# yeyupiaoling/PPASR

Hardware: AMD Instinct MI355X
Metric: audio-seconds/s (RTF^-1) Conformer-streaming fbank, batch32 per GPU, ctc_greedy (higher is better)
Workload: dtype f32; 1 GPU; configs[1]: Conformer streaming (configs/conformer.yml), fbank-80, 32 x 10 s utterances per GPU, V=4233, ctc_greedy, features resident in HBM -> token ids + scores on device; global_batch=32, frames=1000, decoder=ctc_greedy, parallelism=utterance-dp1, pipelined=False, gemm=f32

## Files before the change

### ppasr_amd/csrc/encode_common.h

```cpp
#pragma once

struct RaggedPlan {
  bool skip;
  const int64_t* lens;
  int rc;
  bool rate_changes;
  int mul0;
  int slack(int mul) const { return rate_changes && mul == mul0 ? 2 * (rc + 4) + rc + 8 : rc + 4; }
  PadSkip at(int Tcur, int mul) const {
    PadSkip ps;
    if (skip) {
      ps.lens = lens;
      ps.Tp = Tcur;
      ps.mul = mul;
      ps.slack = slack(mul);
    }
    return ps;
  }
  int attn_pad_skip(const PadSkip& ps) const { return skip ? ps.slack + 1 : 0; }
};

struct BlockTables {
  struct Tab { int Ti, R; int* tab; } tabs[4];
  int n = 0, B;
  bool fits, on;
  size_t off, cap;
  int* base;
  hipStream_t st;
  BlockTables(bool skip, int B_, int M, float* stats, hipStream_t st_)
      : B(B_), off(((size_t)B_ + 2 + 15) / 16 * 16), cap(2 * (((size_t)M + 63) / 64 * 64)), base(reinterpret_cast<int*>(stats)), st(st_) {
    fits = (size_t)B + 2 <= cap / 2;
    on = skip && fits && block_tables_enabled();
  }
  int* tile_tab() const { return fits ? base : nullptr; }
  PadSkip make(PadSkip p, int Tcur, int R) {
    const size_t len = 1 + ((size_t)B * Tcur + R - 1) / R;
    if (!on || n == 4 || off + len > cap) return p;
    int* t = base + off;
    launch_block_table(p, B * Tcur, R, t, st);
    tabs[n++] = Tab{Tcur, R, t};
    off += (len + 15) / 16 * 16;
    p.tab = t;
    return p;
  }
  PadSkip with_table(PadSkip p, int Tcur, int R) {
    for (int k = 0; k < n; ++k)
      if (tabs[k].Ti == Tcur && tabs[k].R == R) {
        p.tab = tabs[k].tab;
        return p;
      }
    return make(p, Tcur, R);
  }
};

struct Taps {
  float* buf;
  size_t cap;
  hipStream_t st;
  size_t off = 0;
  void operator()(const float* src, size_t n_floats) {
    if (buf && off + n_floats <= cap)
      (void)hipMemcpyAsync(buf + off, src, n_floats * sizeof(float), hipMemcpyDeviceToDevice, st);
    off += n_floats;
  }
};

struct NoSpans {
  template <typename Fn>
  void operator()(int, Fn&& fn) const { fn(); }
};

template <typename Spans>
inline void front4_fused(const ppasr_model_s* h, const float* feats, int B, int T, const PadSkip& ps, int* tile_tab,
                         bool scale_before_bias, int embed_slices, const PadSkip& ps_embed, float* y1, float* y2, float* xa,
                         hipStream_t st, Spans&& spans) {
  const auto fd = h->front_dims(T);
  const int F = h->desc.input_dim, T1 = fd.T1, F1 = h->F1, Tp = fd.Tp, F2 = h->F2;
  const bool il4 = h->desc.input_layer == 0;
  const f32x4* conv2_h3 = h->gemm_mode == PPASR_GEMM_F16X3 ? h->conv2_w_h3 : nullptr;
  const bool conv12 = il4 && !conv2_h3 && conv12_enabled(h) && conv12_supported(h->front, F, F2);
  if (!conv12) spans(0, [&] { launch_conv1(feats, h->front, y1, B, T, F, T1, F1, st, ps); });
  spans(1, [&] {
    if (conv12) launch_conv12(feats, h->front, y2, B, T, F, Tp, F2, st, ps, tile_tab);
    else if (il4 && !conv2_h3 && conv2_quad_supported(h->front)) launch_conv2_quad(y1, h->front, y2, B, T1, F1, Tp, F2, st, ps, tile_tab);
    else launch_conv2(y1, h->front, y2, B, T1, F1, Tp, F2, st, ps, tile_tab, il4 ? conv2_h3 : nullptr);
  });
  spans(2, [&] {
    launch_embed(y2, h->front, xa, B * Tp, F2 * kD, sqrtf((float)kD), scale_before_bias, st, ps_embed, embed_slices, y1,
                 conv2_h3 ? h->embed_w_h3 : nullptr);
  });
}

inline ppasr_status memory_out(const ppasr_model_s* h, const float* x, const float* g, const float* b, int M, int D,
                               const PadSkip& ps, hipStream_t st) {
  if (!h->memory_out) return PPASR_OK;
  if ((size_t)M * D > h->memory_floats) return fail(PPASR_ENOSPACE, "memory buffer too small (ppasr_set_memory_out)");
  launch_memory_out(x, g, b, h->memory_out, M, D, ps, st);
  return PPASR_OK;
}

template <typename Spans>
inline ppasr_status fused_head_tail(const ppasr_model_s* h, const float* x, float* probs, float* logits, int32_t* frame_argmax,
                                    float* frame_maxprob, float* ws, const WsLayout& wl, int B, int M, int slices,
                                    const PadSkip& ps, hipStream_t st, Spans&& spans) {
  if (ppasr_status ms = memory_out(h, x, h->head.ln_g, h->head.ln_b, M, kD, ps, st)) return ms;
  float* lg = logits ? logits : probs;
  int32_t* fa = frame_argmax ? frame_argmax : reinterpret_cast<int32_t*>(ws + wl.fa);
  float* fp = frame_maxprob ? frame_maxprob : ws + wl.fp;
  spans(7, [&] {
    const bool head_h3 = h->gemm_mode == PPASR_GEMM_F16X3 && h->head_w_h3;
    HeadW hw = h->head;
    if (head_h3) hw.w = h->head_w_h3;
    launch_ctc_head(x, hw, lg, fa, fp, ws + wl.rmax, ws + wl.rsum, M, st, ps, slices, ws + wl.y1, head_h3);
  });
  if (probs) {
    if (logits) HIP_TRY(hipMemcpyAsync(probs, logits, (size_t)M * h->head.V * sizeof(float), hipMemcpyDeviceToDevice, st));
    launch_softmax_from_stats(probs, ws + wl.rmax, ws + wl.rsum, M, h->head.V, st, ps);
  }
  if (ps.lens) launch_zero_pad_rows(probs, logits, fa, fp, ps.lens, B, ps.Tp, ps.mul, h->head.V, st);
  HIP_TRY(hipGetLastError());
  return PPASR_OK;
}

struct LayerRoute {
  int form;
  int S;
  bool fuse_attn;
  bool h3, h3s;
};
inline bool fuse_rows(const ppasr_model_s* h, int rows) {
  constexpr int fuse_min_blocks = 128;
  return ffn_split_for(h, rows) == 1 && (h->ffn_split == 0 || (rows + kRows - 1) / kRows > fuse_min_blocks);
}
inline LayerRoute layer_route(const ppasr_model_s* h, int B, int Ti, int mul, int slack, bool skip, int layer) {
  const int Mi = B * Ti;
  LayerRoute r;
  const int rows = (!h->taps && conv_ffn_16_supported(h->layer_ks[layer], Ti)) ? row_block_for(h, B, Ti, mul, slack, skip) : 32;
  const bool r16 = rows == 16 && h->ffn_split < 0;
  r.fuse_attn = !r16 && h->layer_group[layer] == 1 && h->desc.attention_heads == 4 && !h->taps && fuse_rows(h, Mi);
  r.S = r16 ? 1 : ffn_split_for(h, Mi);
  const bool w16 = rows == kW16 && r.S == 1;
  r.form = r16 ? 16 : w16 ? kW16 : 32;
  r.h3 = h->h3_layers() && !r16 && !w16 && r.S == 1;
  r.h3s = h->h3_layers() && r.S > 1;
  return r;
}
```

### ppasr_amd/csrc/front_fused.hip

```cpp
#include <utility>

#include "conformer_kernels.h"
#include "launch.h"

namespace ppasr {

namespace {
constexpr int kGroupRow[5] = {2, 0, 1, 4, 3};
constexpr int kTapCol[5] = {2, 0, 1, 4, 3};
constexpr int kFactor[5] = {2, 0, 1, 3, 1};
constexpr int quad_slab(int t) { return 4 * kFactor[t / 5] + kFactor[t % 5]; }
constexpr int quad_target(int t) {
  const int g = t / 5, k = t % 5;
  if (g == 0) return k == 0 ? 4 : k <= 2 ? 5 : 4;
  const int a = (g == 1 || g == 2) ? 0 : 2;
  return k == 0 ? (a == 0 ? 5 : 4) : k <= 2 ? a : a + 1;
}
constexpr int quad_fold_src(int t) {
  return t == 1 || t == 5 || t == 21 || t == 23 ? 4 : t == 3 || t == 11 || t == 13 ? 5 : -1;
}
constexpr int quad_fold_mask(int t) {
  return t == 1 ? 0xf : t == 3 ? 0x5 : t == 5 ? 0xa : t == 11 ? 0x2 : t == 13 ? 0x1 : t == 21 ? 0x8 : t == 23 ? 0x4 : 0;
}
constexpr bool quad_fold_clear(int t) { return t == 1 || t == 3 || t == 5 || t == 13 || t == 23; }
static_assert(quad_target(0) == 4 && quad_target(2) == 5 && quad_target(10) == 5 && quad_target(12) == 0 &&
                  quad_target(14) == 1 && quad_target(20) == 4 && quad_target(22) == 2 && quad_target(24) == 3,
              "chunk targets");

template <typename Fn, int... I>
__device__ __forceinline__ void static_for(std::integer_sequence<int, I...>, Fn&& fn) {
  (fn(std::integral_constant<int, I>{}), ...);
}

__host__ __device__ inline int quad_xs_stride(int F, int Q) { return F > 8 * Q + 3 ? F : 8 * Q + 3; }
}

template <bool FROM_Y1>
__device__ __forceinline__ void conv2_quad_body(const float* __restrict__ src, const FrontW& fw, float* __restrict__ out,
                                                int T, int F, int Tp, int F2, int M, int m0, const PadSkip& ps,
                                                const int* __restrict__ tile_tab) {
  constexpr int BP = 32, KC = 128, LD = KC + 4, G = KC / 8, NL = 2, N_CHUNKS = 25;
  constexpr int SLOT = BP * LD;
  const int P = (Tp + 1) >> 1;
  const int Q = (F2 + 1) >> 1;
  int r0 = m0 + blockIdx.x * BP, Mlim = M;
  if (tile_tab) {
    const int t = blockIdx.x, nb = tile_tab[0];
    const int* pre = tile_tab + 1;
    if (t >= pre[nb]) return;
    int lo = 0, hi = nb;
    while (hi - lo > 1) {
      const int mid = (lo + hi) >> 1;
      if (pre[mid] <= t) lo = mid;
      else hi = mid;
    }
    const int S = ps.Tp * ps.unit;
    r0 = lo * S + (t - pre[lo]) * BP;
    Mlim = min(M, (lo + 1) * S);
  } else if (pad_block_skippable(ps, r0, BP, M)) {
    return;
  }
  extern __shared__ __attribute__((aligned(16))) float smem[];
  float* const slot0 = smem;
  float* const slot1 = smem + SLOT;
  f32x4* const y2s = reinterpret_cast<f32x4*>(smem + 2 * SLOT);
  float* const w1s = smem + 2 * SLOT + 5 * NL * 4 * kThreads;
  float* const xs = w1s + 10 * 256;
  const int tid = threadIdx.x, lane = lane_id(), wave = wave_id();
  constexpr int tile_stride = 2 * 16 * G * 64;
  const f32x4* wbase = fw.conv2_wp + (size_t)wave * tile_stride;
  auto seg = [&](int h, int slab) { return wbase + (size_t)(16 * h + slab) * G * 64; };
  BRing<1> ring;
  ring_prime(ring, seg(0, quad_slab(0)), 0);
  const int c4 = tid & 31, rbase = tid >> 5;
  const int bp0 = r0 / Q;
  const int FX = quad_xs_stride(F, Q);
  uint32_t pb = 0;
  int yrow[FROM_Y1 ? NL : 1], yp4[FROM_Y1 ? NL : 1], yq4[FROM_Y1 ? NL : 1];
  if constexpr (!FROM_Y1) {
    for (int idx = tid; idx < 10 * 256; idx += kThreads) w1s[idx] = idx < 9 * 256 ? fw.conv1_w[idx] : fw.conv1_b[idx - 9 * 256];
    const int nbp = (min(r0 + BP, Mlim) - 1) / Q - bp0 + 1;
    for (int idx = tid; idx < nbp * 11 * FX; idx += kThreads) {
      const int fr_row = idx / FX, f = idx - fr_row * FX;
      const int bpl = fr_row / 11, fr = fr_row - 11 * bpl;
      const int bp = bp0 + bpl, b = bp / P, p = bp - b * P;
      const int t = min(8 * p + fr, T - 1);
      xs[idx] = f < F ? (src[((size_t)b * T + t) * F + f] - fw.cmvn_mean[f]) * fw.cmvn_istd[f] : 0.f;
    }
#pragma unroll
    for (int i = 0; i < NL; ++i) {
      const int m = r0 + rbase + 16 * i;
      const int bp = m / Q, q = m - bp * Q;
      const uint32_t v = m < Mlim ? (uint32_t)((bp - bp0) * 11 * FX + 8 * q) : 0xffffu;
      pb |= v << (16 * i);
    }
  } else {
#pragma unroll
    for (int i = 0; i < NL; ++i) {
      const int m = r0 + rbase + 16 * i;
      const int bp = m / Q, q = m - bp * Q, b = bp / P, p = bp - b * P;
      yrow[i] = b * T + 4 * p;
      yp4[i] = 4 * p;
      yq4[i] = m < Mlim ? 4 * q : -1;
    }
  }
  auto pbase = [&](int i) { return (int)((pb >> (16 * i)) & 0xffffu); };
  const int lds_off0 = rbase * LD + 4 * c4;
  float xv[9];
  f32x4 wv[3], bv, ya, yv;
  auto y1_step = [&](int i, int h, int r, int c, int step) {
    const int cc = h * 128 + 4 * c4;
    if constexpr (!FROM_Y1) {
      if (step == 0) {
        const int o = pbase(i);
        const float* p = xs + (o == 0xffff ? 0 : o) + 2 * r * FX + 2 * c;
#pragma unroll
        for (int ii = 0; ii < 3; ++ii)
#pragma unroll
          for (int jj = 0; jj < 3; ++jj) xv[ii * 3 + jj] = p[ii * FX + jj];
        ya = f32x4{0.f, 0.f, 0.f, 0.f};
      } else {
#pragma unroll
        for (int j = 3 * (step - 1); j < 3 * step; ++j)
#pragma unroll
          for (int e = 0; e < 4; ++e) ya[e] = fmaf(wv[j % 3][e], xv[j], ya[e]);
        if (step == 3) {
          ya += bv;
#pragma unroll
          for (int e = 0; e < 4; ++e) ya[e] = pbase(i) != 0xffff ? fmaxf(ya[e], 0.f) : 0.f;
        }
      }
      if (step < 3) {
#pragma unroll
        for (int j = 0; j < 3; ++j) wv[j] = *reinterpret_cast<const f32x4*>(w1s + (3 * step + j) * 256 + cc);
        if (step == 2) bv = *reinterpret_cast<const f32x4*>(w1s + 9 * 256 + cc);
      }
    } else {
      if (step == 0) {
        yv = f32x4{0.f, 0.f, 0.f, 0.f};
        if (yq4[i] >= 0 && yp4[i] + r < T && yq4[i] + c < F)
          yv = *reinterpret_cast<const f32x4*>(src + ((size_t)(yrow[i] + r) * F + yq4[i] + c) * 256 + cc);
      } else if (step == 3) {
        ya = yv;
      }
    }
  };
  auto put = [&](float* buf, int i, const f32x4& v) { *reinterpret_cast<f32x4*>(buf + lds_off0 + i * 16 * LD) = v; };
  auto y2row = [&](int c, int i) -> f32x4& { return y2s[(c * NL + i) * kThreads + tid]; };
  f32x4 z2[NL];
  auto build = [&](auto nc, int g, int h, float* buf) {
    constexpr int n = decltype(nc)::value, grp = n / 5, k = n % 5, r = kGroupRow[grp], c = kTapCol[k];
    const int i = g >> 2, step = g & 3;
    y1_step(i, h, r, c, step);
    if (step != 3) return;
    f32x4 v = ya;
    if constexpr (grp == 0) y2row(c, i) = ya;
    if constexpr (grp == 1 || grp == 3) v = ya - y2row(c, i);
    if constexpr (k == 0) {
      z2[i] = v;
      put(buf, i, v);
    } else if constexpr (k == 1 || k == 3) {
      put(buf, i, v - z2[i]);
    } else {
      put(buf, i, v);
    }
  };
  f32x16 acc[6][1][1];
#pragma unroll
  for (int a = 0; a < 6; ++a) acc_zero(acc[a]);
  auto fold = [&](auto tc, int g) {
    constexpr int t = decltype(tc)::value, fs = quad_fold_src(t), mask = quad_fold_mask(t);
    if constexpr (fs >= 0) {
      const int j = g - 4 * NL;
      int seen = 0;
#pragma unroll
      for (int o = 0; o < 4; ++o) {
        if (!((mask >> o) & 1)) continue;
        if (seen++ == j) {
#pragma unroll
          for (int e = 0; e < 16; ++e) asm volatile("v_add_f32 %0, %0, %1" : "+v"(acc[o][0][0][e]) : "v"(acc[fs][0][0][e]));
        }
      }
      if (quad_fold_clear(t) && j == 4) acc_zero(acc[fs]);
    }
  };
  __syncthreads();
#pragma unroll
  for (int g = 0; g < 4 * NL; ++g) {
    build(std::integral_constant<int, 0>{}, g, 0, slot0);
    __builtin_amdgcn_sched_barrier(0);
  }
  __syncthreads();
  for (int h = 0; h < 2; ++h) {
    asm volatile("" : "+s"(wbase));
    if constexpr (!FROM_Y1) {
      asm volatile("" : "+v"(pb));
    } else {
#pragma unroll
      for (int i = 0; i < NL; ++i) asm volatile("" : "+v"(yrow[i]), "+v"(yp4[i]), "+v"(yq4[i]));
    }
    static_for(std::make_integer_sequence<int, N_CHUNKS>{}, [&](auto tc) {
      constexpr int t = decltype(tc)::value;
      float* const cur = ((t + h) & 1) ? slot1 : slot0;
      float* const nxb = ((t + h) & 1) ? slot0 : slot1;
      const f32x4* nseg = t + 1 < N_CHUNKS ? seg(h, quad_slab(t + 1)) : (h == 0 ? seg(1, quad_slab(0)) : nullptr);
      auto side = [&](int g) {
        if (g < 4 * NL) {
          if constexpr (t + 1 < N_CHUNKS) build(std::integral_constant<int, t + 1>{}, g, h, nxb);
          else if (h == 0) build(std::integral_constant<int, 0>{}, g, 1, nxb);
        } else {
          fold(tc, g);
        }
      };
      rb_gemm<1, 1, G, kPF, decltype(side)>(cur, LD, seg(h, quad_slab(t)), 0, nseg, 0, ring, acc[quad_target(t)], side);
      __syncthreads();
    });
  }
  const int col = wave * 32 + (lane & 31);
  const float b2 = fw.conv2_b[col];
#pragma unroll
  for (int r = 0; r < 16; ++r) {
    const int m = r0 + acc_row(r, lane);
    if (m >= Mlim) continue;
    const int bp = m / Q, q = m - bp * Q, b = bp / P, t0 = 2 * (bp - b * P), f0 = 2 * q;
    float* o = out + ((size_t)(b * Tp + t0) * F2 + f0) * 256 + col;
    const bool f1 = f0 + 1 < F2, t1 = t0 + 1 < Tp;
    o[0] = fmaxf(acc[0][0][0][r] + b2, 0.f);
    if (f1) o[256] = fmaxf(acc[1][0][0][r] + b2, 0.f);
    if (t1) o[(size_t)F2 * 256] = fmaxf(acc[2][0][0][r] + b2, 0.f);
    if (t1 && f1) o[(size_t)F2 * 256 + 256] = fmaxf(acc[3][0][0][r] + b2, 0.f);
  }
}

__global__ __launch_bounds__(kThreads) void k_conv12(const float* __restrict__ feats, FrontW fw, float* __restrict__ out,
                                                     int T, int F, int Tp, int F2, int M, int m0, PadSkip ps,
                                                     const int* __restrict__ tile_tab) {
  conv2_quad_body<false>(feats, fw, out, T, F, Tp, F2, M, m0, ps, tile_tab);
}
__global__ __launch_bounds__(kThreads) void k_conv2_pair(const float* __restrict__ y1, FrontW fw, float* __restrict__ out,
                                                         int T1, int F1, int Tp, int F2, int M, int m0, PadSkip ps,
                                                         const int* __restrict__ tile_tab) {
  conv2_quad_body<true>(y1, fw, out, T1, F1, Tp, F2, M, m0, ps, tile_tab);
}

static int quad_tile_pairs(int Q) { return 31 / Q + 2; }
static size_t quad_lds(bool fused, int F, int F2) {
  const int Q = (F2 + 1) / 2;
  return ((size_t)2 * 32 * 132 + (size_t)5 * 2 * 4 * 512 + (fused ? (size_t)10 * 256 + (size_t)quad_tile_pairs(Q) * 11 * quad_xs_stride(F, Q) : 0)) *
         sizeof(float);
}
bool conv2_quad_supported(const FrontW& fw) { return fw.conv2_wp && fw.conv2_k == 3 && fw.conv2_s == 2; }
bool conv12_supported(const FrontW& fw, int F, int F2) {
  const int Q = (F2 + 1) / 2;
  return conv2_quad_supported(fw) && F2 >= 1 && quad_lds(true, F, F2) <= 160 * 1024 &&
         (size_t)quad_tile_pairs(Q) * 11 * quad_xs_stride(F, Q) < 0xffff;
}

void launch_tile_prefix(const PadSkip& ps, int B, int BM, int* tab, hipStream_t st);

static void launch_quad(bool fused, const float* src, const FrontW& fw, float* y2, int B, int T, int F, int Tp, int F2,
                        hipStream_t st, const PadSkip& ps_frames, int* tile_scratch) {
  const int P = (Tp + 1) / 2, Q = (F2 + 1) / 2;
  PadSkip ps = ps_frames;
  ps.Tp = P;
  ps.mul = 2 * ps_frames.mul;
  ps.slack = (ps_frames.slack + 1) / 2;
  ps.unit = Q;
  const int M = B * P * Q;
  const int* no_tab = nullptr;
#define QUAD(GRID, TAB)                                                                                                  \
  do {                                                                                                                 \
    if (fused)                                                                                                         \
      PPASR_LAUNCH(k_conv12, dim3(GRID), dim3(kThreads), quad_lds(true, F, F2), st, src, fw, y2, T, F, Tp, F2, M, 0, ps, \
                   TAB);                                                                                               \
    else                                                                                                               \
      PPASR_LAUNCH(k_conv2_pair, dim3(GRID), dim3(kThreads), quad_lds(false, F, F2), st, src, fw, y2, T, F, Tp, F2, M, 0, \
                   ps, TAB);                                                                                           \
  } while (0)
  if (ps.lens && tile_scratch) {
    launch_tile_prefix(ps, B, 32, tile_scratch, st);
    QUAD(B * ((P * Q + 31) / 32), (const int*)tile_scratch);
    return;
  }
  QUAD((M + 31) / 32, no_tab);
#undef QUAD
}

void launch_conv12(const float* feats, const FrontW& fw, float* y2, int B, int T, int F, int Tp, int F2, hipStream_t st,
                   const PadSkip& ps_frames, int* tile_scratch) {
  launch_quad(true, feats, fw, y2, B, T, F, Tp, F2, st, ps_frames, tile_scratch);
}
void launch_conv2_quad(const float* y1, const FrontW& fw, float* y2, int B, int T1, int F1, int Tp, int F2, hipStream_t st,
                       const PadSkip& ps_frames, int* tile_scratch) {
  launch_quad(false, y1, fw, y2, B, T1, F1, Tp, F2, st, ps_frames, tile_scratch);
}

hipError_t configure_front_fused_kernels() {
  hipError_t e;
#define SET_LDS(fn)                                                                                              \
  e = hipFuncSetAttribute(reinterpret_cast<const void*>(fn), hipFuncAttributeMaxDynamicSharedMemorySize, 160 * 1024); \
  if (e != hipSuccess) return e;
  SET_LDS(k_conv12);
  SET_LDS(k_conv2_pair);
#undef SET_LDS
  return hipSuccess;
}

}
```

### ppasr_amd/csrc/front_kernels.hip

```cpp
#include <algorithm>
#include <cstdlib>

#include "conformer_kernels.h"
#include "launch.h"
#include "phases.h"
#include "h3.h"

#include <math.h>

namespace ppasr {
#ifdef PPASR_PHASE_TS
}
extern "C" __attribute__((visibility("default"))) int ppasr_debug_read_wave_ts_front(long long* out) {
  return (int)hipMemcpyFromSymbol(out, HIP_SYMBOL(ppasr::g_wave_ts), sizeof(long long) * 512);
}
namespace ppasr {
#endif

__global__ void k_posproj(const float* __restrict__ pe, const float* __restrict__ wpos,
                          const float* __restrict__ bpos, float* __restrict__ ptab, int max_len, int d) {
  int pos = blockIdx.x;
  int n = threadIdx.x;
  __shared__ float row[1024];
  row[n] = pe[(size_t)pos * d + n];
// ... 80 lines not shown
  constexpr int BM = 32 * MT;
  int r0_map = 0, Mlim = M;
  if (tile_tab) {
    const int t = blockIdx.x, nb = tile_tab[0];
    const int* pre = tile_tab + 1;
    if (t >= pre[nb]) return;
    int lo = 0, hi = nb;
    while (hi - lo > 1) {
      const int mid = (lo + hi) >> 1;
      if (pre[mid] <= t) lo = mid;
      else hi = mid;
    }
    const int S = ps.Tp * ps.unit;
    r0_map = lo * S + (t - pre[lo]) * BM;
    Mlim = min(M, (lo + 1) * S);
  } else if (ps.tab) {
    const int blk = pad_block_of(ps, BM, M);
    if (blk < 0) return;
    r0_map = blk * BM;
  } else if (pad_block_skippable(ps, m0 + blockIdx.x * BM, BM, M)) {
    return;
  }
  constexpr int LD = H3 ? (KC + 8) / 2 : KC + 4;
  constexpr int LDH = KC + 8, PLANE = BM * LDH;
  constexpr int BUF = H3 ? PLANE : BM * LD;
  constexpr int F4_PER_ROW = KC / 4;
  constexpr int NL = BM * F4_PER_ROW / kThreads;
  constexpr int G = KC / 8;
  extern __shared__ __attribute__((aligned(16))) float smem[];
  const int tid = threadIdx.x, lane = lane_id(), wave = wave_id();
  const int r0 = (tile_tab || ps.tab) ? r0_map : m0 + blockIdx.x * BM;
  const int tile_stride = n_chunks * G * 64;
  const int kc0 = (int)((long long)blockIdx.z * n_chunks / gridDim.z), kc1 = (int)((long long)(blockIdx.z + 1) * n_chunks / gridDim.z);
  const f32x4* wbase = wp + (size_t)(blockIdx.y * kWaves + wave) * tile_stride;
  BRing<1> ring;
  ring_prime(ring, wbase + (size_t)kc0 * G * 64, 0);
  const float* tile_base = src.base(min(r0, M - 1));
  const __amdgpu_buffer_rsrc_t rs_a = wstream_rsrc(tile_base);
  int voff[NL];
  int lds_off[NL];
#pragma unroll
  for (int i = 0; i < NL; ++i) {
    int idx = tid + kThreads * i;
    int row = idx / F4_PER_ROW, c4 = idx - row * F4_PER_ROW;
    int m = r0 + row;
    voff[i] = (m < Mlim) ? (int)((src.base(m) - tile_base) * sizeof(float)) + 16 * c4 : 0x7fffffff;
    lds_off[i] = H3 ? row * LDH + 4 * c4 : row * LD + 4 * c4;
  }
  f32x4 stg[NL];
  auto load_chunk = [&](int kc) {
    const int soff = (int)(src.chunk_off(kc) * sizeof(float));
#pragma unroll
    for (int i = 0; i < NL; ++i) stg[i] = wstream_load(rs_a, voff[i], soff);
  };
  bool bad = false;
  auto write_piece = [&](float* buf, int i) {
    _Float16* pl = reinterpret_cast<_Float16*>(buf);
    f16x4 hi, lo;
    h3_split4(stg[i] * kH3Sa, hi, lo, bad);
    *reinterpret_cast<f16x4*>(pl + lds_off[i]) = hi;
    *reinterpret_cast<f16x4*>(pl + PLANE + lds_off[i]) = lo;
  };
  auto write_chunk = [&](float* buf) {
    if constexpr (H3) {
#pragma unroll
      for (int i = 0; i < NL; ++i) write_piece(buf, i);
    } else {
#pragma unroll
      for (int i = 0; i < NL; ++i) *reinterpret_cast<f32x4*>(buf + lds_off[i]) = stg[i];
    }
  };
  f32x16 acc[MT][1];
  acc_zero(acc);
  load_chunk(kc0);
  write_chunk(smem + (kc0 & 1) * BUF);
  __syncthreads();
  for (int kc = kc0; kc < kc1; ++kc) {
    float* cur = smem + (kc & 1) * BUF;
    float* nxt = smem + ((kc + 1) & 1) * BUF;
    const bool more = kc + 1 < kc1;
    if (more) load_chunk(kc + 1);
    const f32x4* seg = wbase + (size_t)kc * G * 64;
    if (MT == 4 && kc < 8) PPASR_WAVE_TS(32 + 4 * kc);
    if constexpr (H3) {
      constexpr int KS = KC / 16, PER = (NL + KS - 1) / KS;
      auto side = [&](int ks) {
        if (more) {
#pragma unroll
          for (int j = 0; j < PER; ++j)
            if (ks * PER + j < NL) write_piece(nxt, ks * PER + j);
        }
      };
      rb_gemm_h3_rows<MT, KS>(reinterpret_cast<const _Float16*>(cur), LDH, PLANE, seg, more ? seg + G * 64 : nullptr, ring, acc,
                              side);
    } else {
      rb_gemm<MT, 1, G>(cur, LD, seg, 0, more ? seg + G * 64 : nullptr, 0, ring, acc);
    }
    if (MT == 4 && kc < 8) PPASR_WAVE_TS(33 + 4 * kc);
    if constexpr (!H3) {
      if (more) write_chunk(nxt);
    }
    if (MT == 4 && kc < 8) PPASR_WAVE_TS(34 + 4 * kc);
    __syncthreads();
    if (MT == 4 && kc < 8) PPASR_WAVE_TS(35 + 4 * kc);
  }
  if constexpr (H3) {
    h3_note(bad);
#pragma unroll
    for (int mt = 0; mt < MT; ++mt) acc[mt][0] *= kH3Inv;
  }
  const int col = blockIdx.y * 256 + wave * 32 + (lane & 31);
  if (gridDim.z > 1) {
    float* po = out + (size_t)blockIdx.z * M * ldc;
#pragma unroll
    for (int mt = 0; mt < MT; ++mt)
#pragma unroll
      for (int r = 0; r < 16; ++r) {
        int m = r0 + mt * 32 + acc_row(r, lane);
        if (m < Mlim && col < n_valid) po[(size_t)m * ldc + col] = acc[mt][0][r];
      }
    return;
  }
  const float bv = bias[col];
#pragma unroll
  for (int mt = 0; mt < MT; ++mt)
#pragma unroll
    for (int r = 0; r < 16; ++r) {
      int m = r0 + mt * 32 + acc_row(r, lane);
      float v = SB ? acc[mt][0][r] * scale + bv : (acc[mt][0][r] + bv) * scale;
      if (RELU) v = fmaxf(v, 0.f);
      if (m < Mlim && col < n_valid) out[(size_t)m * ldc + col] = v;
    }
}
template <int MT, int KC, bool RELU, bool SB, typename Src>
__global__ __launch_bounds__(kThreads) void k_gemm_stream(Src src, const f32x4* __restrict__ wp,
                                                          const float* __restrict__ bias, float* __restrict__ out, int M,
                                                          int n_chunks, float scale, int ldc, int n_valid, int m0,
                                                          PadSkip ps, const int* __restrict__ tile_tab) {
  gemm_stream_body<MT, KC, RELU, SB, Src, false>(src, wp, bias, out, M, n_chunks, scale, ldc, n_valid, m0, ps, tile_tab);
}
template <int MT>
__global__ __launch_bounds__(kThreads) void k_conv_stage_h3(Conv2Src src, const f32x4* __restrict__ wp,
                                                            const float* __restrict__ bias, float* __restrict__ out, int M,
                                                            int n_chunks, float scale, int ldc, int n_valid, int m0, PadSkip ps,
                                                            const int* __restrict__ tile_tab) {
  gemm_stream_body<MT, 128, true, false, Conv2Src, true>(src, wp, bias, out, M, n_chunks, scale, ldc, n_valid, m0, ps, tile_tab);
}
template <bool SB>
__global__ __launch_bounds__(kThreads) void k_embed_h3(DenseSrc src, const f32x4* __restrict__ wp, const float* __restrict__ bias,
                                                       float* __restrict__ out, int M, int n_chunks, float scale, int ldc,
                                                       int n_valid, int m0, PadSkip ps, const int* __restrict__ tile_tab) {
  gemm_stream_body<1, 256, false, SB, DenseSrc, true>(src, wp, bias, out, M, n_chunks, scale, ldc, n_valid, m0, ps, tile_tab);
}
__global__ __launch_bounds__(256) void k_tile_prefix(PadSkip ps, int B, int BM, int* __restrict__ tab) {
  __shared__ int cnt[256];
  int run = 0;
  if (threadIdx.x == 0) {
    tab[0] = B;
    tab[1] = 0;
  }
  for (int b0 = 0; b0 < B; b0 += 256) {
    const int b = b0 + threadIdx.x;
    cnt[threadIdx.x] = b < B ? (pad_need_steps(ps, b) * ps.unit + BM - 1) / BM : 0;
    __syncthreads();
    if (threadIdx.x == 0) {
      for (int i = 0; i < 256 && b0 + i < B; ++i) {
        run += cnt[i];
        tab[2 + b0 + i] = run;
      }
    }
    __syncthreads();
  }
}
__global__ __launch_bounds__(256) void k_block_table(PadSkip ps, int M, int R, int* __restrict__ tab) {
  __shared__ int cnt[256];
  const int nblk = (M + R - 1) / R, tid = threadIdx.x;
  int run = 0;
  for (int b0 = 0; b0 < nblk; b0 += 256) {
    const int i = b0 + tid;
    const int act = (i < nblk && !pad_block_skippable(ps, i * R, R, M)) ? 1 : 0;
    cnt[tid] = act;
    __syncthreads();
    for (int o = 1; o < 256; o <<= 1) {
      const int v = tid >= o ? cnt[tid - o] : 0;
      __syncthreads();
      cnt[tid] += v;
      __syncthreads();
    }
    if (act) tab[1 + run + cnt[tid] - 1] = i;
    run += cnt[255];
    __syncthreads();
  }
  if (tid == 0) tab[0] = run;
}
void launch_block_table(const PadSkip& ps, int M, int R, int* tab, hipStream_t st) {
  PadSkip p = ps;
  p.tab = nullptr;
  PPASR_LAUNCH(k_block_table, dim3(1), dim3(256), 0, st, p, M, R, tab);
}
void launch_tile_prefix(const PadSkip& ps, int B, int BM, int* tab, hipStream_t st) {
  PPASR_LAUNCH(k_tile_prefix, dim3(1), dim3(256), 0, st, ps, B, BM, tab);
}
__global__ __launch_bounds__(256) void k_gemm_join(const float* __restrict__ part, int nz, const float* __restrict__ bias,
                                                   float scale, int scale_before_bias, float* __restrict__ out, int M,
                                                   PadSkip ps) {
  const int row = blockIdx.x * 4 + (threadIdx.x >> 6), lane = threadIdx.x & 63;
  if (row >= M) return;
  if (pad_block_skippable(ps, row & ~(kRows - 1), kRows, M)) return;
  f32x4 acc = *reinterpret_cast<const f32x4*>(part + (size_t)row * kD + 4 * lane);
  for (int z = 1; z < nz; ++z) acc += *reinterpret_cast<const f32x4*>(part + ((size_t)z * M + row) * kD + 4 * lane);
  const f32x4 bv = *reinterpret_cast<const f32x4*>(bias + 4 * lane);
  f32x4 y;
#pragma unroll
  for (int e = 0; e < 4; ++e) {
    y[e] = (scale_before_bias & 1) ? acc[e] * scale + bv[e] : (acc[e] + bv[e]) * scale;
    if (scale_before_bias & 2) y[e] = fmaxf(y[e], 0.f);
  }
  *reinterpret_cast<f32x4*>(out + (size_t)row * kD + 4 * lane) = y;
}
constexpr int kConvSplitMax = 9;
constexpr int kConvSplitRows = 32 * 28;
size_t conv_stage_part_floats(int M, int channels) {
  return (channels == 256 && M <= kConvSplitRows) ? (size_t)kConvSplitMax * M * 256 : 0;
}
size_t conv_stage_part_reserve(int M) { return conv_stage_part_floats(std::min(M, kConvSplitRows)); }

void launch_conv2(const float* y1, const FrontW& fw, float* y2, int B, int T1, int F1, int Tp, int F2, hipStream_t st,
                  const PadSkip& ps_frames, int* tile_scratch, const f32x4* w_h3, float* part, size_t part_floats) {
  launch_conv_stage(y1, w_h3 ? w_h3 : fw.conv2_w, fw.conv2_b, y2, B, T1, F1, Tp, F2, fw.conv2_k, fw.conv2_s, st, ps_frames, 256,
                    tile_scratch, w_h3 != nullptr, part, part_floats);
}
void launch_conv_stage(const float* y1, const f32x4* conv_w, const float* conv_b, float* y2, int B, int T1, int F1, int Tp,
                       int F2, int ksz, int stride, hipStream_t st, const PadSkip& ps_frames, int channels, int* tile_scratch,
                       bool h3, float* part, size_t part_floats) {
  Conv2Src src{y1, T1, F1, Tp, F2, ksz, stride, channels};
  const int n_kc = ksz * ksz * (channels / 128);
  const int ny = channels / 256;
  PadSkip ps = ps_frames;
  ps.unit = F2;
  const int M = B * Tp * F2;
  constexpr int KC = 128, kCUs = 256;
  auto lds_of = [h3](int mt) {
    return h3 ? (size_t)2 * 2 * (32 * mt) * (KC + 8) * sizeof(_Float16) : (size_t)2 * (32 * mt) * (KC + 4) * sizeof(float);
  };
  const int* no_tab = nullptr;
#define CONV_STAGE_LAUNCH(MTX, GRID, M0, TAB)                                                                            \
  do {                                                                                                                    \
    if (h3)                                                                                                               \
      PPASR_LAUNCH((k_conv_stage_h3<MTX>), GRID, dim3(kThreads), lds_of(MTX), st, src, conv_w, conv_b, y2, M, n_kc, 1.0f, \
                   channels, channels, M0, ps, TAB);                                                                      \
    else                                                                                                                  \
      PPASR_LAUNCH((k_gemm_stream<MTX, KC, true, false, Conv2Src>), GRID, dim3(kThreads), lds_of(MTX), st, src, conv_w,   \
                   conv_b, y2, M, n_kc, 1.0f, channels, channels, M0, ps, TAB);                                           \
  } while (0)
  if (ps.lens && tile_scratch && M > 128 * kCUs) {
    PPASR_LAUNCH(k_tile_prefix, dim3(1), dim3(256), 0, st, ps, B, 128, tile_scratch);
    const int per_utt = (Tp * F2 + 127) / 128;
    CONV_STAGE_LAUNCH(4, dim3(B * per_utt, ny), 0, (const int*)tile_scratch);
    return;
  }
  const int tiles4 = (M + 127) / 128;
  const int full = (tiles4 / kCUs) * kCUs;
  const int rem_rows = M - full * 128;
  int mt_rem = (rem_rows + 32 * kCUs - 1) / (32 * kCUs);
  if (full == 0) {
    const int mt = (M + 32 * kCUs - 1) / (32 * kCUs);
    const int tiles = (M + 31) / 32;
    if (part && !h3 && ny == 1 && !ps.lens && tiles <= 28) {
      int z = kConvSplitMax;
      while (z > 1 && (n_kc % z != 0 || tiles * z > kCUs || (size_t)z * M * 256 > part_floats)) --z;
      if (z > 1) {
        PPASR_LAUNCH((k_gemm_stream<1, KC, true, false, Conv2Src>), dim3(tiles, 1, z), dim3(kThreads), lds_of(1), st, src, conv_w,
                     conv_b, part, M, n_kc, 1.0f, channels, channels, 0, ps, no_tab);
        PPASR_LAUNCH(k_gemm_join, dim3((M + 3) / 4), dim3(256), 0, st, part, z, conv_b, 1.0f, 2, y2, M, PadSkip{});
        return;
      }
    }
#define CONV2_ALL(MTA) CONV_STAGE_LAUNCH(MTA, dim3((M + 32 * MTA - 1) / (32 * MTA), ny), 0, no_tab)
    if (mt <= 1) CONV2_ALL(1);
    else if (mt == 2) CONV2_ALL(2);
    else if (mt == 3) CONV2_ALL(3);
    else CONV2_ALL(4);
#undef CONV2_ALL
    return;
  }
  if (rem_rows <= 0 || mt_rem >= 4) {
    CONV_STAGE_LAUNCH(4, dim3(tiles4, ny), 0, no_tab);
    return;
  }
  CONV_STAGE_LAUNCH(4, dim3(full, ny), 0, no_tab);
  const int m0 = full * 128;
#define CONV2_REM(MTR) CONV_STAGE_LAUNCH(MTR, dim3((rem_rows + 32 * MTR - 1) / (32 * MTR), ny), m0, no_tab)
  if (mt_rem <= 1) CONV2_REM(1);
  else if (mt_rem == 2) CONV2_REM(2);
  else CONV2_REM(3);
#undef CONV2_REM
#undef CONV_STAGE_LAUNCH
}
size_t ragged_lds(size_t lds, const PadSkip& ps, int n_blocks) {
  return (ps.lens && n_blocks > 256 && lds < kLdsExclusive) ? kLdsExclusive : lds;
}

void launch_embed(const float* y2, const FrontW& fw, float* x0, int M, int K, float xscale, bool scale_before_bias,
                  hipStream_t st, const PadSkip& ps, int k_slices, float* part, const f32x4* w_h3) {
  constexpr int MT = 1, KC = 256;
  DenseSrc src{y2, K, KC};
  size_t lds = ragged_lds(2 * (32 * MT) * (KC + 4) * sizeof(float), ps, (M + 31) / 32);
  if (w_h3 && !(k_slices > 1 && part)) {
    lds = ragged_lds((size_t)2 * 2 * 32 * (KC + 8) * sizeof(_Float16), ps, (M + 31) / 32);
    if (scale_before_bias)
      PPASR_LAUNCH(k_embed_h3<true>, dim3((M + 31) / 32), dim3(kThreads), lds, st, src, w_h3, fw.embed_b, x0, M, K / KC, xscale,
                   kD, kD, 0, ps, (const int*)nullptr);
    else
      PPASR_LAUNCH(k_embed_h3<false>, dim3((M + 31) / 32), dim3(kThreads), lds, st, src, w_h3, fw.embed_b, x0, M, K / KC, xscale,
                   kD, kD, 0, ps, (const int*)nullptr);
    return;
  }
  if (k_slices > 1 && part) {
    PPASR_LAUNCH((k_gemm_stream<MT, KC, false, false, DenseSrc>), dim3((M + 31) / 32, 1, k_slices), dim3(kThreads), lds,
                       st, src, fw.embed_w, fw.embed_b, part, M, K / KC, xscale, kD, kD, 0, ps, (const int*)nullptr);
    PPASR_LAUNCH(k_gemm_join, dim3((M + 3) / 4), dim3(256), 0, st, part, k_slices, fw.embed_b, xscale,
                       scale_before_bias ? 1 : 0, x0, M, ps);
    return;
  }
  if (scale_before_bias)
    PPASR_LAUNCH((k_gemm_stream<MT, KC, false, true, DenseSrc>), dim3((M + 31) / 32), dim3(kThreads), lds, st, src,
                       fw.embed_w, fw.embed_b, x0, M, K / KC, xscale, kD, kD, 0, ps, (const int*)nullptr);
  else
    PPASR_LAUNCH((k_gemm_stream<MT, KC, false, false, DenseSrc>), dim3((M + 31) / 32), dim3(kThreads), lds, st, src,
                       fw.embed_w, fw.embed_b, x0, M, K / KC, xscale, kD, kD, 0, ps, (const int*)nullptr);
}

__global__ __launch_bounds__(256) void k_dense_join(const float* __restrict__ part, int nz, const float* __restrict__ bias,
                                                    float scale, float* __restrict__ out, int M, int ldc, int n_valid) {
  const size_t i = (size_t)blockIdx.x * 256 + threadIdx.x;
  const int per_row = (n_valid + 3) / 4;
  if (i >= (size_t)M * per_row) return;
  const int m = (int)(i / per_row), c = 4 * (int)(i - (size_t)m * per_row);
  float acc[4] = {0.f, 0.f, 0.f, 0.f};
  for (int z = 0; z < nz; ++z)
#pragma unroll
    for (int e = 0; e < 4; ++e)
      if (c + e < n_valid) acc[e] += part[((size_t)z * M + m) * ldc + c + e];
#pragma unroll
  for (int e = 0; e < 4; ++e)
    if (c + e < n_valid) out[(size_t)m * ldc + c + e] = (acc[e] + bias[c + e]) * scale;
}

void launch_dense(const float* a, int lda, const f32x4* w, const float* bias, float* out, int M, int K, int n_cols_padded,
                  int ldc, int n_valid, hipStream_t st, float scale, float* part, size_t part_floats) {
  constexpr int MT = 1, KC = 256;
  DenseSrc src{a, lda, KC};
  size_t lds = 2 * (32 * MT) * (KC + 4) * sizeof(float);
  const int tiles = ((M + 31) / 32) * (n_cols_padded / 256), n_kc = K / KC;
  int S = 1;
  if (part && tiles <= 128) {
    S = 8;
    while (S > 1 && (tiles * S > 256 || n_kc % S != 0 || (size_t)S * M * ldc > part_floats)) S >>= 1;
  }
  if (S > 1) {
    PPASR_LAUNCH((k_gemm_stream<MT, KC, false, false, DenseSrc>), dim3((M + 31) / 32, n_cols_padded / 256, S), dim3(kThreads),
                 lds, st, src, w, bias, part, M, n_kc, scale, ldc, n_valid, 0, PadSkip{}, (const int*)nullptr);
    const size_t n4 = (size_t)M * ((n_valid + 3) / 4);
    PPASR_LAUNCH(k_dense_join, dim3((unsigned)((n4 + 255) / 256)), dim3(256), 0, st, part, S, bias, scale, out, M, ldc, n_valid);
    return;
  }
  PPASR_LAUNCH((k_gemm_stream<MT, KC, false, false, DenseSrc>), dim3((M + 31) / 32, n_cols_padded / 256),
                     dim3(kThreads), lds, st, src, w, bias, out, M, K / KC, scale, ldc, n_valid, 0, PadSkip{}, (const int*)nullptr);
}

unsigned int* front_h3_ovf_counter() { return h3_ovf_counter(); }

hipError_t configure_front_kernels() {
  hipError_t e = hipSuccess;
#define SET_LDS(fn, bytes)                                                                                     \
  e = hipFuncSetAttribute(reinterpret_cast<const void*>(fn), hipFuncAttributeMaxDynamicSharedMemorySize, (int)(bytes)); \
  if (e != hipSuccess) return e;
  SET_LDS(k_conv_stage_h3<4>, 2 * 2 * 128 * 136 * sizeof(_Float16));
  SET_LDS(k_conv_stage_h3<3>, 2 * 2 * 96 * 136 * sizeof(_Float16));
  SET_LDS(k_conv_stage_h3<2>, 2 * 2 * 64 * 136 * sizeof(_Float16));
  SET_LDS(k_conv_stage_h3<1>, 2 * 2 * 32 * 136 * sizeof(_Float16));
  SET_LDS((k_gemm_stream<4, 128, true, false, Conv2Src>), 2 * 128 * 132 * sizeof(float));
  SET_LDS((k_gemm_stream<3, 128, true, false, Conv2Src>), 2 * 96 * 132 * sizeof(float));
  SET_LDS((k_gemm_stream<2, 128, true, false, Conv2Src>), 2 * 64 * 132 * sizeof(float));
  SET_LDS((k_gemm_stream<1, 128, true, false, Conv2Src>), 2 * 32 * 132 * sizeof(float));
  SET_LDS(k_embed_h3<false>, kLdsExclusive);
  SET_LDS(k_embed_h3<true>, kLdsExclusive);
  SET_LDS((k_gemm_stream<1, 256, false, false, DenseSrc>), kLdsExclusive);
  SET_LDS((k_gemm_stream<1, 256, false, true, DenseSrc>), kLdsExclusive);
#undef SET_LDS
  return hipSuccess;
}

__global__ __launch_bounds__(256) void k_pos_dtab(const float* __restrict__ ptab, const float* __restrict__ pos_u,
                                                  const float* __restrict__ pos_v, float* __restrict__ dtab, int max_len) {
  const int t = blockIdx.x * 256 + threadIdx.x, h = blockIdx.y;
  if (t >= max_len) return;
  double acc = 0.0;
  for (int c = 0; c < 64; ++c)
    acc += ((double)pos_v[64 * h + c] - (double)pos_u[64 * h + c]) * (double)ptab[(size_t)t * 256 + 64 * h + c];
  dtab[(size_t)h * max_len + t] = (float)acc;
}
void launch_pos_dtab(const float* ptab, const float* pos_u, const float* pos_v, float* dtab, int max_len, hipStream_t st) {
  PPASR_LAUNCH(k_pos_dtab, dim3((max_len + 255) / 256, 4), dim3(256), 0, st, ptab, pos_u, pos_v, dtab, max_len);
}

}
```

Baseline: 58480 audio-s/s.

## Split odd-width conv2 quad tiles into main and edge-column kernels

When the subsampled frequency width F2 is odd, the quad conv2 kernel previously computed four outputs per quad, and the last column's f+1 outputs were discarded. The change routes the last frequency column through a separate EDGE path that uses 3 tap chunks instead of 5 and 3 accumulators instead of 6. It adds a second prefix table for the edge tiles so padding skip still works, and enlarges the block-table offset to leave room for it. This trades extra tiles and code complexity for removing wasted GEMM work on the padded half-quad.

```diff
diff --git a/ppasr_amd/csrc/encode_common.h b/ppasr_amd/csrc/encode_common.h
--- a/ppasr_amd/csrc/encode_common.h
+++ b/ppasr_amd/csrc/encode_common.h
@@ -28,7 +28,7 @@
   int* base;
   hipStream_t st;
   BlockTables(bool skip, int B_, int M, float* stats, hipStream_t st_)
-      : B(B_), off(((size_t)B_ + 2 + 15) / 16 * 16), cap(2 * (((size_t)M + 63) / 64 * 64)), base(reinterpret_cast<int*>(stats)), st(st_) {
+      : B(B_), off((2 * ((size_t)B_ + 2) + 15) / 16 * 16), cap(2 * (((size_t)M + 63) / 64 * 64)), base(reinterpret_cast<int*>(stats)), st(st_) {
     fits = (size_t)B + 2 <= cap / 2;
     on = skip && fits && block_tables_enabled();
   }
diff --git a/ppasr_amd/csrc/front_fused.hip b/ppasr_amd/csrc/front_fused.hip
--- a/ppasr_amd/csrc/front_fused.hip
+++ b/ppasr_amd/csrc/front_fused.hip
@@ -33,33 +33,31 @@
 }
 
 __host__ __device__ inline int quad_xs_stride(int F, int Q) { return F > 8 * Q + 3 ? F : 8 * Q + 3; }
-}
-
-template <bool FROM_Y1>
+
+constexpr int edge_slab(int t) { return 4 * kFactor[t / 3] + (t % 3 == 2 ? 3 : t % 3); }
+constexpr int edge_target(int t) { return t < 3 ? 2 : t < 9 ? 0 : 1; }
+constexpr int kEdgeFX = 7;
+static_assert(edge_slab(0) == 8 && edge_slab(2) == 11 && edge_slab(3) == 0 && edge_slab(7) == 5 && edge_slab(11) == 15 &&
+                  edge_slab(13) == 5,
+              "edge slabs");
+
+struct QuadRows {
+  int unit, q_base;
+  __device__ __forceinline__ void at(int m, int& bp, int& ql) const {
+    bp = m / unit;
+    ql = m - bp * unit;
+  }
+};
+}
+
+template <bool FROM_Y1, bool EDGE>
 __device__ __forceinline__ void conv2_quad_body(const float* __restrict__ src, const FrontW& fw, float* __restrict__ out,
-                                                int T, int F, int Tp, int F2, int M, int m0, const PadSkip& ps,
-                                                const int* __restrict__ tile_tab) {
-  constexpr int BP = 32, KC = 128, LD = KC + 4, G = KC / 8, NL = 2, N_CHUNKS = 25;
+                                                int T, int F, int Tp, int F2, int r0, int Mlim, const QuadRows rows) {
+  constexpr int BP = 32, KC = 128, LD = KC + 4, G = KC / 8, NL = 2, NT = EDGE ? 3 : 5, N_CHUNKS = 5 * NT;
   constexpr int SLOT = BP * LD;
   const int P = (Tp + 1) >> 1;
   const int Q = (F2 + 1) >> 1;
-  int r0 = m0 + blockIdx.x * BP, Mlim = M;
-  if (tile_tab) {
-    const int t = blockIdx.x, nb = tile_tab[0];
-    const int* pre = tile_tab + 1;
-    if (t >= pre[nb]) return;
-    int lo = 0, hi = nb;
-    while (hi - lo > 1) {
-      const int mid = (lo + hi) >> 1;
-      if (pre[mid] <= t) lo = mid;
-      else hi = mid;
-    }
-    const int S = ps.Tp * ps.unit;
-    r0 = lo * S + (t - pre[lo]) * BP;
-    Mlim = min(M, (lo + 1) * S);
-  } else if (pad_block_skippable(ps, r0, BP, M)) {
-    return;
-  }
+  auto slab = [](int t) constexpr { return EDGE ? edge_slab(t) : quad_slab(t); };
   extern __shared__ __attribute__((aligned(16))) float smem[];
   float* const slot0 = smem;
   float* const slot1 = smem + SLOT;
@@ -69,19 +67,19 @@
   const int tid = threadIdx.x, lane = lane_id(), wave = wave_id();
   constexpr int tile_stride = 2 * 16 * G * 64;
   const f32x4* wbase = fw.conv2_wp + (size_t)wave * tile_stride;
-  auto seg = [&](int h, int slab) { return wbase + (size_t)(16 * h + slab) * G * 64; };
+  auto seg = [&](int h, int sl) { return wbase + (size_t)(16 * h + sl) * G * 64; };
   BRing<1> ring;
-  ring_prime(ring, seg(0, quad_slab(0)), 0);
+  ring_prime(ring, seg(0, slab(0)), 0);
   const int c4 = tid & 31, rbase = tid >> 5;
-  const int bp0 = r0 / Q;
-  const int FX = quad_xs_stride(F, Q);
+  const int bp0 = r0 / rows.unit;
+  const int FX = EDGE ? kEdgeFX : quad_xs_stride(F, Q);
   uint32_t pb = 0;
   int yrow[FROM_Y1 ? NL : 1], yp4[FROM_Y1 ? NL : 1], yq4[FROM_Y1 ? NL : 1];
   if constexpr (!FROM_Y1) {
     for (int idx = tid; idx < 10 * 256; idx += kThreads) w1s[idx] = idx < 9 * 256 ? fw.conv1_w[idx] : fw.conv1_b[idx - 9 * 256];
-    const int nbp = (min(r0 + BP, Mlim) - 1) / Q - bp0 + 1;
+    const int nbp = (min(r0 + BP, Mlim) - 1) / rows.unit - bp0 + 1;
     for (int idx = tid; idx < nbp * 11 * FX; idx += kThreads) {
-      const int fr_row = idx / FX, f = idx - fr_row * FX;
+      const int fr_row = idx / FX, f = idx - fr_row * FX + 8 * rows.q_base;
       const int bpl = fr_row / 11, fr = fr_row - 11 * bpl;
       const int bp = bp0 + bpl, b = bp / P, p = bp - b * P;
       const int t = min(8 * p + fr, T - 1);
@@ -90,18 +88,21 @@
 #pragma unroll
     for (int i = 0; i < NL; ++i) {
       const int m = r0 + rbase + 16 * i;
-      const int bp = m / Q, q = m - bp * Q;
-      const uint32_t v = m < Mlim ? (uint32_t)((bp - bp0) * 11 * FX + 8 * q) : 0xffffu;
+      int bp, ql;
+      rows.at(m, bp, ql);
+      const uint32_t v = m < Mlim ? (uint32_t)((bp - bp0) * 11 * FX + 8 * ql) : 0xffffu;
       pb |= v << (16 * i);
     }
   } else {
 #pragma unroll
     for (int i = 0; i < NL; ++i) {
       const int m = r0 + rbase + 16 * i;
-      const int bp = m / Q, q = m - bp * Q, b = bp / P, p = bp - b * P;
+      int bp, ql;
+      rows.at(m, bp, ql);
+      const int b = bp / P, p = bp - b * P;
       yrow[i] = b * T + 4 * p;
       yp4[i] = 4 * p;
-      yq4[i] = m < Mlim ? 4 * q : -1;
+      yq4[i] = m < Mlim ? 4 * (rows.q_base + ql) : -1;
     }
   }
   auto pbase = [&](int i) { return (int)((pb >> (16 * i)) & 0xffffu); };
@@ -147,16 +148,18 @@
   };
   auto put = [&](float* buf, int i, const f32x4& v) { *reinterpret_cast<f32x4*>(buf + lds_off0 + i * 16 * LD) = v; };
   auto y2row = [&](int c, int i) -> f32x4& { return y2s[(c * NL + i) * kThreads + tid]; };
-  f32x4 z2[NL];
+  f32x4 z2[EDGE ? 1 : NL];
   auto build = [&](auto nc, int g, int h, float* buf) {
-    constexpr int n = decltype(nc)::value, grp = n / 5, k = n % 5, r = kGroupRow[grp], c = kTapCol[k];
+    constexpr int n = decltype(nc)::value, grp = n / NT, k = n % NT, r = kGroupRow[grp], c = EDGE ? k : kTapCol[k];
     const int i = g >> 2, step = g & 3;
     y1_step(i, h, r, c, step);
     if (step != 3) return;
     f32x4 v = ya;
     if constexpr (grp == 0) y2row(c, i) = ya;
     if constexpr (grp == 1 || grp == 3) v = ya - y2row(c, i);
-    if constexpr (k == 0) {
+    if constexpr (EDGE) {
+      put(buf, i, v);
+    } else if constexpr (k == 0) {
       z2[i] = v;
       put(buf, i, v);
     } else if constexpr (k == 1 || k == 3) {
@@ -165,11 +168,11 @@
       put(buf, i, v);
     }
   };
-  f32x16 acc[6][1][1];
-#pragma unroll
-  for (int a = 0; a < 6; ++a) acc_zero(acc[a]);
+  f32x16 acc[EDGE ? 3 : 6][1][1];
+#pragma unroll
+  for (int a = 0; a < (EDGE ? 3 : 6); ++a) acc_zero(acc[a]);
   auto fold = [&](auto tc, int g) {
-    constexpr int t = decltype(tc)::value, fs = quad_fold_src(t), mask = quad_fold_mask(t);
+    constexpr int t = decltype(tc)::value, fs = EDGE ? -1 : quad_fold_src(t), mask = quad_fold_mask(t);
     if constexpr (fs >= 0) {
       const int j = g - 4 * NL;
       int seen = 0;
@@ -203,7 +206,7 @@
       constexpr int t = decltype(tc)::value;
       float* const cur = ((t + h) & 1) ? slot1 : slot0;
       float* const nxb = ((t + h) & 1) ? slot0 : slot1;
-      const f32x4* nseg = t + 1 < N_CHUNKS ? seg(h, quad_slab(t + 1)) : (h == 0 ? seg(1, quad_slab(0)) : nullptr);
+      const f32x4* nseg = t + 1 < N_CHUNKS ? seg(h, slab(t + 1)) : (h == 0 ? seg(1, slab(0)) : nullptr);
       auto side = [&](int g) {
         if (g < 4 * NL) {
           if constexpr (t + 1 < N_CHUNKS) build(std::integral_constant<int, t + 1>{}, g, h, nxb);
@@ -212,77 +215,136 @@
           fold(tc, g);
         }
       };
-      rb_gemm<1, 1, G, kPF, decltype(side)>(cur, LD, seg(h, quad_slab(t)), 0, nseg, 0, ring, acc[quad_target(t)], side);
+      rb_gemm<1, 1, G, kPF, decltype(side)>(cur, LD, seg(h, slab(t)), 0, nseg, 0, ring,
+                                            acc[EDGE ? edge_target(t) : quad_target(t)], side);
       __syncthreads();
     });
   }
+  static_assert(N_CHUNKS % 2 == 1, "the A slots alternate across the stage boundary");
   const int col = wave * 32 + (lane & 31);
   const float b2 = fw.conv2_b[col];
 #pragma unroll
   for (int r = 0; r < 16; ++r) {
     const int m = r0 + acc_row(r, lane);
     if (m >= Mlim) continue;
-    const int bp = m / Q, q = m - bp * Q, b = bp / P, t0 = 2 * (bp - b * P), f0 = 2 * q;
+    int bp, ql;
+    rows.at(m, bp, ql);
+    const int b = bp / P, t0 = 2 * (bp - b * P), f0 = 2 * (rows.q_base + ql);
     float* o = out + ((size_t)(b * Tp + t0) * F2 + f0) * 256 + col;
-    const bool f1 = f0 + 1 < F2, t1 = t0 + 1 < Tp;
-    o[0] = fmaxf(acc[0][0][0][r] + b2, 0.f);
-    if (f1) o[256] = fmaxf(acc[1][0][0][r] + b2, 0.f);
-    if (t1) o[(size_t)F2 * 256] = fmaxf(acc[2][0][0][r] + b2, 0.f);
-    if (t1 && f1) o[(size_t)F2 * 256 + 256] = fmaxf(acc[3][0][0][r] + b2, 0.f);
-  }
+    const bool t1 = t0 + 1 < Tp;
+    if constexpr (EDGE) {
+      o[0] = fmaxf(acc[0][0][0][r] + acc[2][0][0][r] + b2, 0.f);
+      if (t1) o[(size_t)F2 * 256] = fmaxf(acc[1][0][0][r] + acc[2][0][0][r] + b2, 0.f);
+    } else {
+      const bool f1 = f0 + 1 < F2;
+      o[0] = fmaxf(acc[0][0][0][r] + b2, 0.f);
+      if (f1) o[256] = fmaxf(acc[1][0][0][r] + b2, 0.f);
+      if (t1) o[(size_t)F2 * 256] = fmaxf(acc[2][0][0][r] + b2, 0.f);
+      if (t1 && f1) o[(size_t)F2 * 256 + 256] = fmaxf(acc[3][0][0][r] + b2, 0.f);
+    }
+  }
+}
+
+template <bool FROM_Y1>
+__device__ __forceinline__ void conv2_quad_tile(const float* __restrict__ src, const FrontW& fw, float* __restrict__ out,
+                                                int T, int F, int Tp, int F2, int M, PadSkip ps,
+                                                const int* __restrict__ tile_tab) {
+  constexpr int BP = 32;
+  const int Q = (F2 + 1) >> 1, n_bp = M / Q;
+  const bool odd = F2 & 1;
+  const int unit_main = odd ? Q - 1 : Q;
+  const int M_main = n_bp * unit_main;
+  int t = blockIdx.x, r0, Mlim;
+  bool edge;
+  if (tile_tab) {
+    const int nb = tile_tab[0];
+    const int* pre = tile_tab + 1;
+    edge = t >= pre[nb];
+    if (edge) {
+      if (!odd) return;
+      t -= pre[nb];
+      pre += nb + 2;
+      if (t >= pre[nb]) return;
+    }
+    int lo = 0, hi = nb;
+    while (hi - lo > 1) {
+      const int mid = (lo + hi) >> 1;
+      if (pre[mid] <= t) lo = mid;
+      else hi = mid;
+    }
+    const int S = ps.Tp * (edge ? 1 : unit_main);
+    r0 = lo * S + (t - pre[lo]) * BP;
+    Mlim = (lo + 1) * S;
+  } else {
+    const int n_main = (M_main + BP - 1) / BP;
+    edge = t >= n_main;
+    if (edge) t -= n_main;
+    r0 = t * BP;
+    Mlim = edge ? n_bp : M_main;
+    ps.unit = edge ? 1 : unit_main;
+    if (pad_block_skippable(ps, r0, BP, Mlim)) return;
+  }
+  if (edge) conv2_quad_body<FROM_Y1, true>(src, fw, out, T, F, Tp, F2, r0, Mlim, QuadRows{1, Q - 1});
+  else conv2_quad_body<FROM_Y1, false>(src, fw, out, T, F, Tp, F2, r0, Mlim, QuadRows{unit_main, 0});
 }
 
 __global__ __launch_bounds__(kThreads) void k_conv12(const float* __restrict__ feats, FrontW fw, float* __restrict__ out,
-                                                     int T, int F, int Tp, int F2, int M, int m0, PadSkip ps,
+                                                     int T, int F, int Tp, int F2, int M, PadSkip ps,
                                                      const int* __restrict__ tile_tab) {
-  conv2_quad_body<false>(feats, fw, out, T, F, Tp, F2, M, m0, ps, tile_tab);
+  conv2_quad_tile<false>(feats, fw, out, T, F, Tp, F2, M, ps, tile_tab);
 }
 __global__ __launch_bounds__(kThreads) void k_conv2_pair(const float* __restrict__ y1, FrontW fw, float* __restrict__ out,
-                                                         int T1, int F1, int Tp, int F2, int M, int m0, PadSkip ps,
+                                                         int T1, int F1, int Tp, int F2, int M, PadSkip ps,
                                                          const int* __restrict__ tile_tab) {
-  conv2_quad_body<true>(y1, fw, out, T1, F1, Tp, F2, M, m0, ps, tile_tab);
-}
-
-static int quad_tile_pairs(int Q) { return 31 / Q + 2; }
+  conv2_quad_tile<true>(y1, fw, out, T1, F1, Tp, F2, M, ps, tile_tab);
+}
+
+static int quad_tile_pairs(int unit) { return unit <= 1 ? 32 : 31 / unit + 2; }
+static int quad_main_unit(int F2) { return (F2 & 1) ? F2 / 2 : (F2 + 1) / 2; }
+static size_t quad_xs_floats(int F, int F2) {
+  const int Q = (F2 + 1) / 2, um = quad_main_unit(F2);
+  const size_t main = um ? (size_t)quad_tile_pairs(um) * 11 * quad_xs_stride(F, Q) : 0;
+  const size_t edge = (F2 & 1) ? (size_t)32 * 11 * kEdgeFX : 0;
+  return main > edge ? main : edge;
+}
 static size_t quad_lds(bool fused, int F, int F2) {
-  const int Q = (F2 + 1) / 2;
-  return ((size_t)2 * 32 * 132 + (size_t)5 * 2 * 4 * 512 + (fused ? (size_t)10 * 256 + (size_t)quad_tile_pairs(Q) * 11 * quad_xs_stride(F, Q) : 0)) *
-         sizeof(float);
+  return ((size_t)2 * 32 * 132 + (size_t)5 * 2 * 4 * 512 + (fused ? (size_t)10 * 256 + quad_xs_floats(F, F2) : 0)) * sizeof(float);
 }
 bool conv2_quad_supported(const FrontW& fw) { return fw.conv2_wp && fw.conv2_k == 3 && fw.conv2_s == 2; }
 bool conv12_supported(const FrontW& fw, int F, int F2) {
-  const int Q = (F2 + 1) / 2;
   return conv2_quad_supported(fw) && F2 >= 1 && quad_lds(true, F, F2) <= 160 * 1024 &&
-         (size_t)quad_tile_pairs(Q) * 11 * quad_xs_stride(F, Q) < 0xffff;
-}
-
-void launch_tile_prefix(const PadSkip& ps, int B, int BM, int* tab, hipStream_t st);
+         quad_xs_floats(F, F2) < 0xffff;
+}
+
+void launch_tile_prefix(const PadSkip& ps, int B, int BM, int* tab, hipStream_t st, int unit2);
 
 static void launch_quad(bool fused, const float* src, const FrontW& fw, float* y2, int B, int T, int F, int Tp, int F2,
                         hipStream_t st, const PadSkip& ps_frames, int* tile_scratch) {
   const int P = (Tp + 1) / 2, Q = (F2 + 1) / 2;
+  const bool odd = F2 & 1;
+  const int unit = quad_main_unit(F2);
   PadSkip ps = ps_frames;
   ps.Tp = P;
   ps.mul = 2 * ps_frames.mul;
   ps.slack = (ps_frames.slack + 1) / 2;
-  ps.unit = Q;
+  ps.unit = unit;
   const int M = B * P * Q;
   const int* no_tab = nullptr;
-#define QUAD(GRID, TAB)                                                                                                  \
-  do {                                                                                                                 \
-    if (fused)                                                                                                         \
-      PPASR_LAUNCH(k_conv12, dim3(GRID), dim3(kThreads), quad_lds(true, F, F2), st, src, fw, y2, T, F, Tp, F2, M, 0, ps, \
-                   TAB);                                                                                               \
-    else                                                                                                               \
-      PPASR_LAUNCH(k_conv2_pair, dim3(GRID), dim3(kThreads), quad_lds(false, F, F2), st, src, fw, y2, T, F, Tp, F2, M, 0, \
-                   ps, TAB);                                                                                           \
+#define QUAD(GRID, TAB)                                                                                               \
+  do {                                                                                                              \
+    if (fused)                                                                                                      \
+      PPASR_LAUNCH(k_conv12, dim3(GRID), dim3(kThreads), quad_lds(true, F, F2), st, src, fw, y2, T, F, Tp, F2, M, ps, \
+                   TAB);                                                                                            \
+    else                                                                                                            \
+      PPASR_LAUNCH(k_conv2_pair, dim3(GRID), dim3(kThreads), quad_lds(false, F, F2), st, src, fw, y2, T, F, Tp, F2, M, \
+                   ps, TAB);                                                                                        \
   } while (0)
   if (ps.lens && tile_scratch) {
-    launch_tile_prefix(ps, B, 32, tile_scratch, st);
-    QUAD(B * ((P * Q + 31) / 32), (const int*)tile_scratch);
+    launch_tile_prefix(ps, B, 32, tile_scratch, st, odd ? 1 : -1);
+    QUAD(B * ((P * unit + 31) / 32 + (odd ? (P + 31) / 32 : 0)), (const int*)tile_scratch);
     return;
   }
-  QUAD((M + 31) / 32, no_tab);
+  QUAD((B * P * unit + 31) / 32 + (odd ? (B * P + 31) / 32 : 0), no_tab);
 #undef QUAD
 }
 
diff --git a/ppasr_amd/csrc/front_kernels.hip b/ppasr_amd/csrc/front_kernels.hip
--- a/ppasr_amd/csrc/front_kernels.hip
+++ b/ppasr_amd/csrc/front_kernels.hip
@@ -256,21 +256,32 @@
                                                        int n_valid, int m0, PadSkip ps, const int* __restrict__ tile_tab) {
   gemm_stream_body<1, 256, false, SB, DenseSrc, true>(src, wp, bias, out, M, n_chunks, scale, ldc, n_valid, m0, ps, tile_tab);
 }
-__global__ __launch_bounds__(256) void k_tile_prefix(PadSkip ps, int B, int BM, int* __restrict__ tab) {
-  __shared__ int cnt[256];
-  int run = 0;
+__global__ __launch_bounds__(256) void k_tile_prefix(PadSkip ps, int B, int BM, int* __restrict__ tab, int unit2) {
+  __shared__ int cnt[256], cnt2[256];
+  int run = 0, run2 = 0;
+  int* const tab2 = tab + B + 2;
   if (threadIdx.x == 0) {
     tab[0] = B;
     tab[1] = 0;
+    if (unit2 >= 0) {
+      tab2[0] = B;
+      tab2[1] = 0;
+    }
   }
   for (int b0 = 0; b0 < B; b0 += 256) {
     const int b = b0 + threadIdx.x;
-    cnt[threadIdx.x] = b < B ? (pad_need_steps(ps, b) * ps.unit + BM - 1) / BM : 0;
+    const int need = b < B ? pad_need_steps(ps, b) : 0;
+    cnt[threadIdx.x] = (need * ps.unit + BM - 1) / BM;
+    cnt2[threadIdx.x] = unit2 >= 0 ? (need * unit2 + BM - 1) / BM : 0;
     __syncthreads();
     if (threadIdx.x == 0) {
       for (int i = 0; i < 256 && b0 + i < B; ++i) {
         run += cnt[i];
         tab[2 + b0 + i] = run;
+        if (unit2 >= 0) {
+          run2 += cnt2[i];
+          tab2[2 + b0 + i] = run2;
+        }
       }
     }
     __syncthreads();
@@ -302,8 +313,8 @@
   p.tab = nullptr;
   PPASR_LAUNCH(k_block_table, dim3(1), dim3(256), 0, st, p, M, R, tab);
 }
-void launch_tile_prefix(const PadSkip& ps, int B, int BM, int* tab, hipStream_t st) {
-  PPASR_LAUNCH(k_tile_prefix, dim3(1), dim3(256), 0, st, ps, B, BM, tab);
+void launch_tile_prefix(const PadSkip& ps, int B, int BM, int* tab, hipStream_t st, int unit2) {
+  PPASR_LAUNCH(k_tile_prefix, dim3(1), dim3(256), 0, st, ps, B, BM, tab, unit2);
 }
 __global__ __launch_bounds__(256) void k_gemm_join(const float* __restrict__ part, int nz, const float* __restrict__ bias,
                                                    float scale, int scale_before_bias, float* __restrict__ out, int M,
@@ -358,7 +369,7 @@
                    conv_b, y2, M, n_kc, 1.0f, channels, channels, M0, ps, TAB);                                           \
   } while (0)
   if (ps.lens && tile_scratch && M > 128 * kCUs) {
-    PPASR_LAUNCH(k_tile_prefix, dim3(1), dim3(256), 0, st, ps, B, 128, tile_scratch);
+    PPASR_LAUNCH(k_tile_prefix, dim3(1), dim3(256), 0, st, ps, B, 128, tile_scratch, -1);
     const int per_utt = (Tp * F2 + 127) / 128;
     CONV_STAGE_LAUNCH(4, dim3(B * per_utt, ny), 0, (const int*)tile_scratch);
     return;
```

After: 58510 audio-s/s, median of 2. Within noise of the previous version (+0.0%).
